# rostin79s/TFHE-AES

Hardware: AMD Instinct MI355X
Metric: AES-128 CTR blocks/sec (FHE) (higher is better)
Workload: dtype u64+f64; 1 GPU; configs[2]: 128 CTR blocks per GPU, Server::aes_encrypt 10 rounds (1280 bit-CBS/block), counters pre-incremented client-side; params=PARAM_OPT, blocks_per_gpu=128, total_blocks=128

## Files before the change

include/fheaes.h:

```cpp
#ifndef FHEAES_H
#define FHEAES_H

#include <stddef.h>
#include <stdint.h>

#ifdef __cplusplus
extern "C" {
#endif

#define FHEAES_OK 0
#define FHEAES_ERR_INVALID -1
#define FHEAES_ERR_NOKEYS -2
#define FHEAES_ERR_DEVICE -3
#define FHEAES_ERR_NOMEM -4

#define FHEAES_HOST 0
#define FHEAES_DEVICE 1

typedef struct fheaes_params {
    uint32_t lwe_dimension;
    uint32_t glwe_dimension;
    uint32_t polynomial_size;
    uint32_t pbs_base_log;
    uint32_t pbs_level;
// ... 85 lines not shown
size_t fheaes_packed_words(const fheaes_ctx *ctx, uint64_t m);
int fheaes_pack_bits(fheaes_ctx *ctx, const uint64_t *lwe_in, uint64_t m, uint64_t *glwe_out, int memspace);
int fheaes_unpack_bits(fheaes_ctx *ctx, const uint64_t *glwe_in, uint64_t m, uint64_t *lwe_out, int memspace);

int fheaes_expand_lwe_seeded(fheaes_ctx *ctx, const uint32_t *mask_key, uint64_t first_index, const uint64_t *bodies, uint64_t m,
                             uint64_t *lwe_out, int memspace);

size_t fheaes_packed_words_mod(const fheaes_ctx *ctx, uint64_t m, uint32_t width);
int fheaes_packed_mod_switch(fheaes_ctx *ctx, const uint64_t *glwe_in, uint64_t n_glwe, uint32_t width, uint64_t *out, int memspace);
int fheaes_pack_bits_mod(fheaes_ctx *ctx, const uint64_t *lwe_in, uint64_t m, uint32_t width, uint64_t *out, int memspace);
int fheaes_unpack_bits_mod(fheaes_ctx *ctx, const uint64_t *in, uint64_t m, uint32_t width, uint64_t *lwe_out, int memspace);

#define FHEAES_STAGE_KEYSWITCH 0
#define FHEAES_STAGE_BLIND_ROTATE 1
#define FHEAES_STAGE_PFPKS 2
#define FHEAES_STAGE_GGSW_FFT 3
#define FHEAES_STAGE_VERTICAL_PACKING 4
#define FHEAES_STAGE_LINEAR 5
#define FHEAES_STAGE_COUNT 6
int fheaes_profile_enable(fheaes_ctx *ctx, int on);
int fheaes_profile_reset(fheaes_ctx *ctx);
int fheaes_profile_read(fheaes_ctx *ctx, int stage, double *total_ms, uint64_t *launches, uint64_t *units);

int fheaes_get_twiddles(double *psi_out);
int fheaes_read_bsk_fourier(fheaes_ctx *ctx, uint32_t i, double *out);
int fheaes_k2_launch_plan(uint64_t m, uint32_t cu_count, uint32_t k, int *form, uint64_t *units_main, uint32_t *r_main,
                          uint64_t *units_tail, uint32_t *r_tail);
int fheaes_k2_launch_plan_forms(uint64_t m, uint32_t cu_count, uint32_t k, int allow_pair, int *form, uint64_t *units_main, uint32_t *r_main,
                                uint64_t *units_tail, uint32_t *r_tail);
int fheaes_k2_context_plan(fheaes_ctx *ctx, uint64_t m, int *form, uint64_t *units_main, uint32_t *r_main, uint64_t *units_tail,
                           uint32_t *r_tail, char *kernel, size_t kernel_cap);
int fheaes_k2_set_parking(fheaes_ctx *ctx, int claimed);
int fheaes_k2_set_forms(fheaes_ctx *ctx, int allow_pair, int allow_home);
#define FHEAES_K2_PARK_SLOTS 1024
int fheaes_k2_park_debug(fheaes_ctx *ctx, const uint32_t *initial_owner, int record);
int fheaes_k2_park_read(fheaes_ctx *ctx, uint64_t *fallbacks, uint64_t *violations, uint32_t *owner_out, uint32_t *record_out,
                        uint64_t record_cap, uint64_t *record_n);
const char *fheaes_version(void);

#ifdef __cplusplus
}
#endif
#endif
```

tfhe_aes_amd/_native.py:

```python
from __future__ import annotations

import ctypes
import os
import re
from pathlib import Path

import numpy as np

from . import _build
from .params import CParams, WopbsParameters

HOST, DEVICE = 0, 1
K2_PARK_SLOTS = 1024
STAGES = ("keyswitch", "blind_rotate", "pfpks", "ggsw_fft", "vertical_packing", "linear")

_u64p = ctypes.POINTER(ctypes.c_uint64)
_dp = ctypes.POINTER(ctypes.c_double)
_u32p = ctypes.POINTER(ctypes.c_uint32)
_ctx = ctypes.c_void_p
_c = ctypes

SIGNATURES = {
    "fheaes_create": (_c.c_int, [_c.POINTER(CParams), _c.c_int, _c.POINTER(_ctx)]),
    "fheaes_destroy": (None, [_ctx]),
    "fheaes_last_error": (_c.c_char_p, [_ctx]),
    "fheaes_key_words": (_c.c_size_t, [_ctx, _c.c_int]),
    "fheaes_upload_keys": (_c.c_int, [_ctx, _c.c_void_p, _c.c_void_p, _c.c_void_p, _c.c_int]),
    "fheaes_key_body_words": (_c.c_size_t, [_ctx, _c.c_int]),
    "fheaes_upload_keys_seeded": (_c.c_int, [_ctx, _c.POINTER(_c.c_uint32), _c.c_void_p, _c.c_void_p, _c.c_void_p, _c.c_int]),
    "fheaes_clone_keys": (_c.c_int, [_ctx, _ctx]),
    "fheaes_clone_info": (_c.c_int, [_ctx, _c.POINTER(_c.c_int), _u64p, _dp]),
    "fheaes_noise_level_seen": (_c.c_int, [_ctx, _c.POINTER(_c.c_uint32), _c.POINTER(_c.c_uint32)]),
    "fheaes_set_stream": (_c.c_int, [_ctx, _c.c_void_p]),
    "fheaes_synchronize": (_c.c_int, [_ctx]),
    "fheaes_reserve": (_c.c_int, [_ctx, _c.c_uint64]),
    "fheaes_keyswitch_batch": (_c.c_int, [_ctx, _c.c_void_p, _c.c_uint64, _c.c_void_p, _c.c_int]),
    "fheaes_cbs_pbs_batch": (_c.c_int, [_ctx, _c.c_void_p, _c.c_uint64, _c.c_uint32, _c.c_void_p, _c.c_int]),
    "fheaes_pfpks_batch": (_c.c_int, [_ctx, _c.c_void_p, _c.c_uint64, _c.c_void_p, _c.c_int]),
    "fheaes_forward_fourier_batch": (_c.c_int, [_ctx, _c.c_void_p, _c.c_uint64, _c.c_void_p, _c.c_int]),
    "fheaes_vertical_packing_batch": (_c.c_int, [_ctx, _c.c_void_p, _c.c_uint64, _c.c_uint32, _c.c_void_p, _c.c_uint32,
                                                 _c.c_int, _c.c_void_p, _c.c_int]),
    "fheaes_wopbs_batch": (_c.c_int, [_ctx, _c.c_void_p, _c.c_uint64, _c.c_uint32, _c.c_void_p, _c.c_uint32, _c.c_int,
                                      _c.c_void_p, _c.c_int]),
    "fheaes_gen_lut": (_c.c_int, [_c.c_uint32, _u64p, _u64p]),
    "fheaes_sbox": (_c.c_int, [_ctx, _c.c_void_p, _c.c_uint64, _c.c_int, _c.c_int]),
# ... 10 lines not shown
    "fheaes_aes_decrypt_equivalent_bits": (_c.c_int, [_ctx, _c.c_void_p, _c.c_uint32, _c.c_void_p, _c.c_uint64, _c.c_int]),
    "fheaes_add_scalar": (_c.c_int, [_ctx, _c.c_void_p, _c.c_uint64, _u64p, _c.c_int]),
    "fheaes_aes_encrypt_public_bits": (_c.c_int, [_ctx, _c.c_void_p, _c.c_uint32, _u64p, _c.c_uint64, _c.c_void_p, _c.c_int]),
    "fheaes_aes_ctr_bits": (_c.c_int, [_ctx, _c.c_void_p, _c.c_uint32, _u64p, _c.c_uint64, _u64p, _c.c_uint64, _c.c_void_p, _c.c_int]),
    "fheaes_aes_public_plan": (_c.c_int, [_u64p, _c.c_uint64, _c.c_uint32, _u64p]),
    "fheaes_aes_key_expansion_batch": (_c.c_int, [_ctx, _c.c_void_p, _c.c_uint32, _c.c_uint64, _c.c_void_p, _c.c_int]),
    "fheaes_aes_decryption_round_keys_batch": (_c.c_int, [_ctx, _c.c_void_p, _c.c_uint32, _c.c_uint64, _c.c_void_p, _c.c_int]),
    "fheaes_aes_encrypt_keyed": (_c.c_int, [_ctx, _c.c_void_p, _c.c_uint32, _c.c_uint64, _u32p, _c.c_void_p, _c.c_uint64, _c.c_int]),
    "fheaes_aes_decrypt_keyed": (_c.c_int, [_ctx, _c.c_void_p, _c.c_uint32, _c.c_uint64, _u32p, _c.c_void_p, _c.c_uint64, _c.c_int]),
    "fheaes_aes_decrypt_equivalent_keyed": (_c.c_int, [_ctx, _c.c_void_p, _c.c_uint32, _c.c_uint64, _u32p, _c.c_void_p, _c.c_uint64, _c.c_int]),
    "fheaes_aes_public_keyed": (_c.c_int, [_ctx, _c.c_void_p, _c.c_uint32, _c.c_uint64, _u32p, _u64p, _u64p, _c.c_uint64, _c.c_void_p, _c.c_int]),
    "fheaes_aes_public_plan_keyed": (_c.c_int, [_u64p, _u32p, _c.c_uint64, _c.c_uint64, _c.c_uint32, _u64p]),
    "fheaes_packed_words": (_c.c_size_t, [_ctx, _c.c_uint64]),
    "fheaes_pack_bits": (_c.c_int, [_ctx, _c.c_void_p, _c.c_uint64, _c.c_void_p, _c.c_int]),
    "fheaes_unpack_bits": (_c.c_int, [_ctx, _c.c_void_p, _c.c_uint64, _c.c_void_p, _c.c_int]),
    "fheaes_expand_lwe_seeded": (_c.c_int, [_ctx, _u32p, _c.c_uint64, _c.c_void_p, _c.c_uint64, _c.c_void_p, _c.c_int]),
    "fheaes_packed_words_mod": (_c.c_size_t, [_ctx, _c.c_uint64, _c.c_uint32]),
    "fheaes_packed_mod_switch": (_c.c_int, [_ctx, _c.c_void_p, _c.c_uint64, _c.c_uint32, _c.c_void_p, _c.c_int]),
    "fheaes_pack_bits_mod": (_c.c_int, [_ctx, _c.c_void_p, _c.c_uint64, _c.c_uint32, _c.c_void_p, _c.c_int]),
    "fheaes_unpack_bits_mod": (_c.c_int, [_ctx, _c.c_void_p, _c.c_uint64, _c.c_uint32, _c.c_void_p, _c.c_int]),
    "fheaes_profile_enable": (_c.c_int, [_ctx, _c.c_int]),
    "fheaes_profile_reset": (_c.c_int, [_ctx]),
    "fheaes_profile_read": (_c.c_int, [_ctx, _c.c_int, _dp, _u64p, _u64p]),
    "fheaes_get_twiddles": (_c.c_int, [_dp]),
    "fheaes_read_bsk_fourier": (_c.c_int, [_ctx, _c.c_uint32, _dp]),
    "fheaes_k2_launch_plan": (_c.c_int, [_c.c_uint64, _c.c_uint32, _c.c_uint32, _c.POINTER(_c.c_int), _c.POINTER(_c.c_uint64), _c.POINTER(_c.c_uint32),
                                       _c.POINTER(_c.c_uint64), _c.POINTER(_c.c_uint32)]),
    "fheaes_k2_launch_plan_forms": (_c.c_int, [_c.c_uint64, _c.c_uint32, _c.c_uint32, _c.c_int, _c.POINTER(_c.c_int), _c.POINTER(_c.c_uint64),
                                             _c.POINTER(_c.c_uint32), _c.POINTER(_c.c_uint64), _c.POINTER(_c.c_uint32)]),
    "fheaes_k2_context_plan": (_c.c_int, [_ctx, _c.c_uint64, _c.POINTER(_c.c_int), _c.POINTER(_c.c_uint64), _c.POINTER(_c.c_uint32),
                                        _c.POINTER(_c.c_uint64), _c.POINTER(_c.c_uint32), _c.c_char_p, _c.c_size_t]),
    "fheaes_k2_set_parking": (_c.c_int, [_ctx, _c.c_int]),
    "fheaes_k2_set_forms": (_c.c_int, [_ctx, _c.c_int, _c.c_int]),
    "fheaes_k2_park_debug": (_c.c_int, [_ctx, _c.POINTER(_c.c_uint32), _c.c_int]),
    "fheaes_k2_park_read": (_c.c_int, [_ctx, _u64p, _u64p, _c.POINTER(_c.c_uint32), _c.POINTER(_c.c_uint32), _c.c_uint64, _u64p]),
    "fheaes_version": (_c.c_char_p, []),
}

_lib = None


def header_symbols() -> list[str]:
    text = (_build.ROOT / "include" / "fheaes.h").read_text()
    text = re.sub(r"/\*.*?\*/", "", text, flags=re.S)
    return sorted(set(re.findall(r"\b(fheaes_[a-z0-9_]+)\s*\(", text)))


def load_library(build: bool = True):
    global _lib
    if _lib is not None:
        return _lib
    path = _build.build_engine() if build else _build.ENGINE_SO
    try:
        import torch
    except ImportError:
        pass
    if not Path(path).exists():
        raise RuntimeError("libfheaes.so is missing: run __graft_entry__.build() (hipcc --offload-arch=gfx950)")
    lib = ctypes.CDLL(str(path))
    for name, (res, args) in SIGNATURES.items():
        fn = getattr(lib, name)
        fn.restype, fn.argtypes = res, args
    _lib = lib
    return lib


# ... 230 lines not shown
    def pack_bits_mod(self, lwe_in, m: int, width: int, out):
        self._check(self._lib.fheaes_pack_bits_mod(self._h, _ptr(lwe_in)[0], m, width, _ptr(out)[0], self._space(lwe_in, out)))

    def unpack_bits_mod(self, packed_in, m: int, width: int, lwe_out):
        self._check(self._lib.fheaes_unpack_bits_mod(self._h, _ptr(packed_in)[0], m, width, _ptr(lwe_out)[0], self._space(packed_in, lwe_out)))

    def profile_enable(self, on: bool = True):
        self._check(self._lib.fheaes_profile_enable(self._h, int(on)))

    def profile_reset(self):
        self._check(self._lib.fheaes_profile_reset(self._h))

    def profile_read(self) -> dict:
        out = {}
        for i, name in enumerate(STAGES):
            ms, launches, units = ctypes.c_double(), ctypes.c_uint64(), ctypes.c_uint64()
            self._check(self._lib.fheaes_profile_read(self._h, i, ctypes.byref(ms), ctypes.byref(launches), ctypes.byref(units)))
            out[name] = {"ms": ms.value, "launches": launches.value, "units": units.value}
        return out

    def k2_plan(self, bits: int) -> dict:
        form, um, rm, ut, rt = _c.c_int(), _c.c_uint64(), _c.c_uint32(), _c.c_uint64(), _c.c_uint32()
        name = _c.create_string_buffer(96)
        self._check(self._lib.fheaes_k2_context_plan(self._h, bits, _c.byref(form), _c.byref(um), _c.byref(rm), _c.byref(ut), _c.byref(rt), name, len(name)))
        return {"form": form.value, "kernel": name.value.decode(), "units_main": um.value, "r_main": rm.value,
                "units_tail": ut.value, "r_tail": rt.value}

    def k2_set_parking(self, claimed: bool):
        self._check(self._lib.fheaes_k2_set_parking(self._h, 1 if claimed else 0))

    def k2_set_forms(self, allow_pair: bool = True, allow_home: bool = True):
        self._check(self._lib.fheaes_k2_set_forms(self._h, 1 if allow_pair else 0, 1 if allow_home else 0))

    def k2_park_debug(self, initial=None, record: bool = False):
        ptr = None
        if initial is not None:
            pat = np.ascontiguousarray(np.asarray(initial, dtype=np.uint32))
            if pat.shape != (K2_PARK_SLOTS,):
                raise ValueError("initial owner words: expected %d, got shape %s" % (K2_PARK_SLOTS, pat.shape))
            ptr = pat.ctypes.data_as(_c.POINTER(_c.c_uint32))
        self._check(self._lib.fheaes_k2_park_debug(self._h, ptr, 1 if record else 0))

    def k2_park_read(self) -> dict:
        fb, vi, n = _c.c_uint64(), _c.c_uint64(), _c.c_uint64()
        u32p = _c.POINTER(_c.c_uint32)
        self._check(self._lib.fheaes_k2_park_read(self._h, None, None, None, None, 0, _c.byref(n)))
        owner = np.zeros(K2_PARK_SLOTS, dtype=np.uint32)
        rec = np.zeros((n.value, 2), dtype=np.uint32)
        self._check(self._lib.fheaes_k2_park_read(self._h, _c.byref(fb), _c.byref(vi), owner.ctypes.data_as(u32p), rec.ctypes.data_as(u32p),
                                                  n.value, _c.byref(n)))
        return {"fallbacks": fb.value, "violations": vi.value, "owner": owner, "record": rec[:n.value]}

    def read_bsk_fourier(self, i: int) -> np.ndarray:
        p = self.params
        out = np.empty((p.pbs_level, p.k + 1, p.k + 1, 256, 2), dtype=np.float64)
        self._check(self._lib.fheaes_read_bsk_fourier(self._h, i, out.ctypes.data_as(_dp)))
        return out


def u128_pairs(values) -> np.ndarray:
    out = np.zeros((len(values), 2), dtype=np.uint64)
    for i, v in enumerate(values):
        if isinstance(v, (bytes, bytearray)):
            if len(v) != 16:
                raise ValueError("an AES block has 16 bytes, got %d" % len(v))
            v = int.from_bytes(v, "big")
# ... 4 lines not shown
    return out


def key_indices(key_of_block, n_blocks: int) -> np.ndarray:
    idx = [int(k) for k in key_of_block]
    if len(idx) != n_blocks:
        raise ValueError("one key index per block expected: %d for %d blocks" % (len(idx), n_blocks))
    if any(not 0 <= k < 1 << 32 for k in idx):
        raise ValueError("a key index is a uint32")
    out = np.zeros(max(n_blocks, 1), dtype=np.uint32)
    out[:n_blocks] = idx
    return out


def aes_public_plan_keyed(blocks, key_of_block, n_keys: int, key_bits: int = 128) -> list[int]:
    cnt = u128_pairs(blocks)
    kob = key_indices(key_of_block, len(cnt))
    out = np.zeros(14, dtype=np.uint64)
    rc = load_library().fheaes_aes_public_plan_keyed(cnt.ctypes.data_as(_u64p), kob.ctypes.data_as(_u32p), len(cnt), n_keys, key_bits, out.ctypes.data_as(_u64p))
    if rc != 0:
        raise FheAesError(rc, "fheaes_aes_public_plan_keyed: key_bits must be 128, 192 or 256, n_keys in 1..65536 and every key index below n_keys")
    return [int(x) for x in out[:{128: 10, 192: 12, 256: 14}[key_bits]]]


def aes_public_plan(blocks, key_bits: int = 128) -> list[int]:
    cnt = u128_pairs(blocks)
    out = np.zeros(14, dtype=np.uint64)
    rc = load_library().fheaes_aes_public_plan(cnt.ctypes.data_as(_u64p), len(cnt), key_bits, out.ctypes.data_as(_u64p))
    if rc != 0:
        raise FheAesError(rc, "fheaes_aes_public_plan: key_bits must be 128, 192 or 256")
    return [int(x) for x in out[:{128: 10, 192: 12, 256: 14}[key_bits]]]


def get_twiddles() -> np.ndarray:
    out = np.empty((512, 2), dtype=np.float64)
    rc = load_library().fheaes_get_twiddles(out.ctypes.data_as(_dp))
    if rc != 0:
        raise FheAesError(rc, "fheaes_get_twiddles")
    return out


def gen_lut(nb_block: int, f_table) -> np.ndarray:
    f = np.ascontiguousarray(f_table, dtype=np.uint64)
    if f.size != 1 << nb_block:
        raise ValueError("f_table must have 2^nb_block entries")
    out = np.empty((nb_block, max(512, 1 << nb_block)), dtype=np.uint64)
    rc = load_library().fheaes_gen_lut(nb_block, f.ctypes.data_as(_u64p), out.ctypes.data_as(_u64p))
    if rc != 0:
        raise FheAesError(rc, "fheaes_gen_lut")
    return out
```

tfhe_aes_amd/csrc/aes_schedule.h:

```cpp
#pragma once

static int many_sbox_dev(fheaes_ctx *c, const uint64_t *bytes, uint64_t n_bytes, int set, uint64_t *out)
{
    return wopbs_dev(c, bytes, n_bytes, 8, c->lutset_d[set], (uint32_t)c->lutset_n[set], 0, out);
}

static int aes_rounds(uint32_t key_bits) { return key_bits == 128 ? 10 : key_bits == 192 ? 12 : key_bits == 256 ? 14 : 0; }

static int check_key_bits(fheaes_ctx *c, uint32_t key_bits)
{
    if (!aes_rounds(key_bits)) return c->fail(FHEAES_ERR_INVALID, "key_bits must be 128, 192 or 256, got %u", key_bits);
    return FHEAES_OK;
}

static int aes_encrypt_dev(fheaes_ctx *c, const KeySets &rk, uint64_t *state, uint64_t n_blocks, int nr)
{
    const uint64_t bw = 8ull * c->big1, sw = 16 * bw, nbytes = 16 * n_blocks;
    TRY(ensure(c, c->ws_vp, nbytes * 3 * bw * 8));
    uint64_t *vp = (uint64_t *)c->ws_vp.p;
    const GatherTable t_round = table_enc_round(), t_shift = table_shift_rows(false);
    TRY(launch_add_bcast(c, state, rk, sw, n_blocks));
    for (int round = 1; round < nr; ++round) {
        TRY(many_sbox_dev(c, state, nbytes, LUTSET_ENC_ROUND, vp));
        TRY(launch_gather(c, vp, 3, rk.round(round, sw), state, n_blocks, t_round));
    }
    TRY(many_sbox_dev(c, state, nbytes, LUTSET_SBOX, vp));
    TRY(launch_gather(c, vp, 1, rk.round(nr, sw), state, n_blocks, t_shift));
    return FHEAES_OK;
}

static int aes_decrypt_dev(fheaes_ctx *c, const KeySets &rk, uint64_t *state, uint64_t n_blocks, int nr)
{
    const uint64_t bw = 8ull * c->big1, sw = 16 * bw, nbytes = 16 * n_blocks;
    TRY(ensure(c, c->ws_vp, nbytes * 4 * bw * 8));
    uint64_t *vp = (uint64_t *)c->ws_vp.p;
    const GatherTable t_inv = table_shift_rows(true), t_mix = table_dec_mix();
    const KeySets no_key{nullptr, nullptr, 0};
    TRY(launch_add_bcast(c, state, rk.round(nr, sw), sw, n_blocks));
    for (int round = nr; round >= 2; --round) {
        TRY(many_sbox_dev(c, state, nbytes, LUTSET_INV_SBOX, vp));
        TRY(launch_gather(c, vp, 1, rk.round(round - 1, sw), state, n_blocks, t_inv));
        TRY(many_sbox_dev(c, state, nbytes, LUTSET_DEC_MUL, vp));
        TRY(launch_gather(c, vp, 4, no_key, state, n_blocks, t_mix));
    }
    TRY(many_sbox_dev(c, state, nbytes, LUTSET_INV_SBOX, vp));
    TRY(launch_gather(c, vp, 1, rk, state, n_blocks, t_inv));
    return FHEAES_OK;
}

static int aes_decrypt_eq_dev(fheaes_ctx *c, const KeySets &dw, uint64_t *state, uint64_t n_blocks, int nr)
{
    const uint64_t bw = 8ull * c->big1, sw = 16 * bw, nbytes = 16 * n_blocks;
    TRY(ensure(c, c->ws_vp, nbytes * 4 * bw * 8));
    uint64_t *vp = (uint64_t *)c->ws_vp.p;
    const GatherTable t_round = table_dec_eq_round(), t_inv = table_shift_rows(true);
    TRY(launch_add_bcast(c, state, dw.round(nr, sw), sw, n_blocks));
    for (int round = nr - 1; round >= 1; --round) {
        TRY(many_sbox_dev(c, state, nbytes, LUTSET_DEC_EQ_ROUND, vp));
        TRY(launch_gather(c, vp, 4, dw.round(round, sw), state, n_blocks, t_round));
    }
    TRY(many_sbox_dev(c, state, nbytes, LUTSET_INV_SBOX, vp));
    TRY(launch_gather(c, vp, 1, dw, state, n_blocks, t_inv));
    return FHEAES_OK;
}

typedef int (*AesDevFn)(fheaes_ctx *, const KeySets &, uint64_t *, uint64_t, int);

static int dec_round_keys_dev(fheaes_ctx *c, const uint64_t *w, uint64_t *dw, int nr, uint64_t n_keys)
{
    const uint64_t bw = 8ull * c->big1, sw = 16 * bw, ks = (uint64_t)(nr + 1) * sw, mid = (uint64_t)(nr - 1) * 16, nbytes = mid * n_keys;
    const bool strided = n_keys > 1;
    TRY(ensure(c, c->ws_vp, nbytes * 4 * bw * 8));
    TRY(ensure(c, c->ws_tmp_a, nbytes * bw * 8));
    if (strided) TRY(ensure(c, c->ws_tmp_b, nbytes * bw * 8));
    uint64_t *vp = (uint64_t *)c->ws_vp.p, *mix = (uint64_t *)c->ws_tmp_a.p, *flat = (uint64_t *)c->ws_tmp_b.p;
    TRY(launch_key_rows(c, dw, ks, w, ks, 0, nullptr, 0, 0, 16, n_keys, 1));
    TRY(launch_key_rows(c, dw + (uint64_t)nr * sw, ks, w + (uint64_t)nr * sw, ks, 0, nullptr, 0, 0, 16, n_keys, 1));
    if (strided) TRY(launch_key_rows(c, flat, mid * bw, w + sw, ks, 0, nullptr, 0, 0, (uint32_t)mid, n_keys, 1));
    TRY(many_sbox_dev(c, strided ? flat : w + sw, nbytes, LUTSET_DEC_MUL, vp));
    TRY(launch_gather(c, vp, 4, KeySets{nullptr, nullptr, 0}, mix, nbytes / 16, table_dec_mix()));
    TRY(many_sbox_dev(c, mix, nbytes, LUTSET_IDENTITY, strided ? flat : dw + sw));
    if (strided) TRY(launch_key_rows(c, dw + sw, ks, flat, mid * bw, 0, nullptr, 0, 0, (uint32_t)mid, n_keys, 1));
    return FHEAES_OK;
}

static int key_expansion_dev(fheaes_ctx *c, const uint64_t *key, uint64_t *w, int nr, uint64_t n_keys)
{
    static const uint8_t RCON[10] = {0x01, 0x02, 0x04, 0x08, 0x10, 0x20, 0x40, 0x80, 0x1B, 0x36};
    const uint64_t bw = 8ull * c->big1, ww = 4 * bw, ks = (uint64_t)(nr + 1) * 16 * bw;
    const int nk = nr - 6;
    const bool strided = n_keys > 1;
    TRY(ensure(c, c->ws_tmp_a, n_keys * ww * 8));
    TRY(ensure(c, c->ws_tmp_b, n_keys * ww * 8));
    if (strided) TRY(ensure(c, c->ws_tmp_c, n_keys * ww * 8));
    uint64_t *ta = (uint64_t *)c->ws_tmp_a.p, *tb = (uint64_t *)c->ws_tmp_b.p, *tc = (uint64_t *)c->ws_tmp_c.p;
    TRY(launch_key_rows(c, w, ks, key, (uint64_t)nk * ww, 0, nullptr, 0, 0, 4u * nk, n_keys, 1));
    for (int i = nk; i < 4 * (nr + 1); ++i) {
// ... 181 lines not shown
```

tfhe_aes_amd/csrc/engine.hip:

```cpp
#include <hip/hip_runtime.h>
#include <cmath>
#include <cstdarg>
#include <cstdio>
#include <atomic>
#include <chrono>
#include <cstring>
#include <mutex>
#include <string>
#include <type_traits>
#include <unordered_map>
#include <vector>

#include "knobs.h"
#include "fheaes.h"
#include "fft_dev.h"
#include "kern_extprod.h"
#include "kern_blindrot_latency.h"
#include "kern_blindrot16.h"
#include "kern_blindrot_pair.h"
#include "ks_launch.h"
#include "kern_linear.h"

#define FHEAES_VERSION_STR "fheaes-mi355x 0.4 (gfx950)" FHEAES_BUILD_KIND

// ... 39 lines not shown
    *form = pl.form; *units_main = pl.units_main; *r_main = pl.r_main; *units_tail = pl.units_tail; *r_tail = pl.r_tail;
    return FHEAES_OK;
}
int fheaes_k2_context_plan(fheaes_ctx *ctx, uint64_t m, int *form, uint64_t *units_main, uint32_t *r_main, uint64_t *units_tail,
                           uint32_t *r_tail, char *kernel, size_t kernel_cap)
{
    if (!ctx) return FHEAES_ERR_INVALID;
    CtxLock lock__(ctx);
    if (!form || !units_main || !r_main || !units_tail || !r_tail || m == 0) return ctx->fail(FHEAES_ERR_INVALID, "k2_context_plan: null output or empty batch");
    const K2Launch L = k2_launch(ctx, m);
    const K2Plan &pl = L.pl;
    *form = pl.form; *units_main = pl.units_main; *r_main = pl.r_main; *units_tail = pl.units_tail; *r_tail = pl.r_tail;
    if (kernel && kernel_cap) { std::strncpy(kernel, L.name, kernel_cap - 1); kernel[kernel_cap - 1] = 0; }
    return FHEAES_OK;
}
int fheaes_k2_set_parking(fheaes_ctx *ctx, int claimed)
{
    if (!ctx) return FHEAES_ERR_INVALID;
    CtxLock lock__(ctx);
    if (claimed != 0 && claimed != 1) return ctx->fail(FHEAES_ERR_INVALID, "k2_set_parking: 1 = claimed slots, 0 = one private slot per workgroup (got %d)", claimed);
    HIP_TRY(ctx, hipStreamSynchronize(ctx->stream));
    ctx->k2_park_claim = claimed;
    return FHEAES_OK;
}
int fheaes_k2_set_forms(fheaes_ctx *ctx, int allow_pair, int allow_home)
{
    if (!ctx) return FHEAES_ERR_INVALID;
    CtxLock lock__(ctx);
    if ((allow_pair != 0 && allow_pair != 1) || (allow_home != 0 && allow_home != 1))
        return ctx->fail(FHEAES_ERR_INVALID, "k2_set_forms: each of allow_pair, allow_home is 0 or 1 (got %d, %d)", allow_pair, allow_home);
    HIP_TRY(ctx, hipStreamSynchronize(ctx->stream));
    ctx->k2_deny_pair = allow_pair == 0;
    ctx->k2_deny_home = allow_home == 0;
    return FHEAES_OK;
}
int fheaes_k2_park_debug(fheaes_ctx *ctx, const uint32_t *initial_owner, int record)
{
    if (!ctx) return FHEAES_ERR_INVALID;
    CtxLock lock__(ctx);
    if (record != 0 && record != 1) return ctx->fail(FHEAES_ERR_INVALID, "k2_park_debug: record must be 0 or 1 (got %d)", record);
    HIP_TRY(ctx, hipSetDevice(ctx->device));
    HIP_TRY(ctx, hipStreamSynchronize(ctx->stream));
    if (initial_owner) {
        TRY(ensure(ctx, ctx->ws_park_pattern, BRP_PARK_SLOTS * sizeof(uint32_t)));
        HIP_TRY(ctx, hipMemcpy(ctx->ws_park_pattern.p, initial_owner, BRP_PARK_SLOTS * sizeof(uint32_t), hipMemcpyHostToDevice));
    }
    if (ctx->ws_park_owner.p)
        HIP_TRY(ctx, hipMemset((char *)ctx->ws_park_owner.p + PARK_RECORD_PTR_OFFSET, 0, sizeof(uint64_t)));
    ctx->k2_park_pattern = initial_owner != nullptr;
    ctx->k2_park_record = record == 1;
    ctx->k2_park_record_n = 0;
    return FHEAES_OK;
}
int fheaes_k2_park_read(fheaes_ctx *ctx, uint64_t *fallbacks, uint64_t *violations, uint32_t *owner_out, uint32_t *record_out,
                        uint64_t record_cap, uint64_t *record_n)
{
    if (!ctx) return FHEAES_ERR_INVALID;
    CtxLock lock__(ctx);
    if (record_out && record_cap < ctx->k2_park_record_n)
        return ctx->fail(FHEAES_ERR_INVALID, "k2_park_read: %llu records do not fit record_cap = %llu", (unsigned long long)ctx->k2_park_record_n,
                         (unsigned long long)record_cap);
    HIP_TRY(ctx, hipSetDevice(ctx->device));
    HIP_TRY(ctx, hipStreamSynchronize(ctx->stream));
    uint32_t words[PARK_OWNER_BYTES / sizeof(uint32_t)] = {};
    if (ctx->ws_park_owner.p) HIP_TRY(ctx, hipMemcpy(words, ctx->ws_park_owner.p, PARK_OWNER_BYTES, hipMemcpyDeviceToHost));
    uint64_t counters[2];
// ... 873 lines not shown
```

tfhe_aes_amd/csrc/engine_ctx.h:

```cpp
#pragma once

namespace {

std::string g_create_error;
thread_local std::string tl_error;
thread_local uint64_t tl_error_ctx_id = 0;
std::atomic<uint64_t> g_next_ctx_id{1};

}

struct DevBuf {
    void *p = nullptr;
    size_t bytes = 0;
    DevBuf() = default;
    DevBuf(const DevBuf &) = delete;
    DevBuf &operator=(const DevBuf &) = delete;
    ~DevBuf() { if (p) (void)hipFree(p); }
};

struct fheaes_ctx {
    fheaes_params p{};
    const uint64_t id = g_next_ctx_id.fetch_add(1);
    int device = 0;
    hipStream_t own_stream = nullptr, stream = nullptr;
    std::string err;
    std::recursive_mutex mu;
    uint32_t n = 0, k = 0, k1 = 0, big = 0, big1 = 0;
    uint32_t cu_count = 256;
    int clone_path = FHEAES_CLONE_NONE;
    uint64_t clone_bytes = 0;
    double clone_seconds = 0.0;
    uint32_t noise_level_seen = 0;
    int k2_home = -1;
    int k2_pair_ok = -1;
    bool k2_deny_pair = false, k2_deny_home = false;
    int k2_park_claim = 1;
    bool k2_park_pattern = false, k2_park_record = false;
    uint64_t k2_park_record_n = 0;
    int8_t *ksk_frag = nullptr, *pfpksk_frag = nullptr;
    uint32_t ks_ksteps = 0, ks_coltiles = 0, pf_ksteps = 0, pf_coltiles = 0;
    size_t ksk_frag_bytes = 0, pfpksk_frag_bytes = 0, bskf_bytes = 0;
    double2 *bskf = nullptr;
    bool have_keys = false;
    double2 *tw_d = nullptr;
    uint64_t *lutset_d[LUTSET_COUNT] = {};
    int lutset_n[LUTSET_COUNT] = {};
    DevBuf ws_small, ws_pbs, ws_ggsw, ws_ggswf, ws_vp, ws_tmp_a, ws_tmp_b, ws_tmp_c, ws_luts, ws_misc, ws_digits, ws_park, ws_park_owner, ws_tree;
    DevBuf ws_park_pattern, ws_park_record;
    DevBuf stage[4];
    uint8_t *pin = nullptr;
    size_t pin_bytes = 0;
    hipEvent_t pin_ev = nullptr;
    bool prof = false;
    struct Pending { hipEvent_t a, b; int stage; };
    std::vector<Pending> pending;
    std::vector<hipEvent_t> free_events;
    double stage_ms[FHEAES_STAGE_COUNT] = {};
    uint64_t stage_launches[FHEAES_STAGE_COUNT] = {};
    uint64_t stage_units[FHEAES_STAGE_COUNT] = {};

    int fail(int code, const char *fmt, ...)
    {
        char buf[512];
        va_list ap;
        va_start(ap, fmt);
        vsnprintf(buf, sizeof buf, fmt, ap);
        va_end(ap);
        err = buf;
        tl_error = buf;
        tl_error_ctx_id = id;
        return code;
// ... 145 lines not shown
```

tfhe_aes_amd/csrc/engine_launch.h:

```cpp
#pragma once

#define MAX_CHUNK_BITS 32768ull
#define MAX_WOPBS_BITS 16u

namespace {

#define LATENCY_BATCH_BITS 256ull
#define K2_PAIR_MIN_BITS 768ull
struct K2Plan { int form; uint64_t units_main; uint32_t r_main; uint64_t units_tail; uint32_t r_tail; };
K2Plan k2_plan(uint64_t m, uint32_t cu_count, uint32_t k1, bool allow_pair = true)
{
    K2Plan pl{};
    if (m <= LATENCY_BATCH_BITS) { pl.form = 0; pl.units_main = m; pl.r_main = 1; return pl; }
    if (allow_pair && k1 == 5 && m > K2_PAIR_MIN_BITS) {
        pl.form = 2; pl.r_main = 6; pl.r_tail = 4;
        const uint64_t gens = (m + 6ull * cu_count - 1) / (6ull * cu_count);
        uint64_t nu = gens * cu_count;
        uint64_t four = 6 * nu >= m ? (6 * nu - m) / 2 : 0;
        if (four > nu) four = nu;
        if (four == nu && 4 * nu > m) { nu = (m + 3) / 4; four = nu; }
        pl.units_tail = four; pl.units_main = nu - four;
        return pl;
    }
    pl.form = 1;
    pl.r_main = k1 == 5 ? 3 : 8;
    pl.units_main = (m + pl.r_main - 1) / pl.r_main;
    if (k1 == 5) {
        const uint64_t slots = 2ull * cu_count;
        pl.r_tail = 2;
        if ((m + 1) / 2 <= cu_count) {
            pl.units_main = 0;
            pl.units_tail = (m + 1) / 2;
        } else if (pl.units_main > slots) {
            const uint64_t nu = slots * ((m + 3 * slots - 1) / (3 * slots));
            if (2 * nu <= m) {
                pl.units_tail = 3 * nu - m;
                pl.units_main = nu - pl.units_tail;
            }
        }
    }
    return pl;
}

int launch_keyswitch(fheaes_ctx *c, const uint64_t *in, uint64_t m, uint64_t *out)
{
    if (m == 0) return FHEAES_OK;
    StageScope sc(c, FHEAES_STAGE_KEYSWITCH, m);
    const uint64_t ct_tiles16 = ((m + KS_CT_TILE - 1) / KS_CT_TILE) * (KS_CT_TILE / 16);
    TRY(ensure(c, c->ws_digits, ct_tiles16 * c->ks_ksteps * 1024));
    int8_t *af = (int8_t *)c->ws_digits.p;
    const uint64_t threads = ct_tiles16 * c->ks_ksteps * 64;
    ks_launch_digits_k1(dim3((unsigned)((threads + 255) / 256)), c->stream, in, (uint64_t)c->big1, c->big, m, c->ks_ksteps, af);
    KeyswitchArgs a{};
    a.afrag = af; a.bfrag = c->ksk_frag; a.ksteps = c->ks_ksteps; a.coltiles = c->ks_coltiles;
    a.in = in; a.in_stride = c->big1; a.body_index = (int32_t)c->big; a.body_col = c->n; a.ncols = c->n + 1;
    a.out = out; a.out_stride = c->n + 1; a.out_z_stride = 0; a.m = m;
    dim3 grid((c->ks_coltiles + KSL_COL_TILES - 1) / KSL_COL_TILES, (unsigned)((m + 16 * KSL_CT_TILES - 1) / (16 * KSL_CT_TILES)), 1);
    ks_launch_mfma_lds(1, grid, c->stream, a);
    HIP_TRY(c, hipGetLastError());
    return FHEAES_OK;
}

int launch_pfpks(fheaes_ctx *c, const uint64_t *in, uint64_t m, uint64_t *out, uint64_t out_stride, int block = -1)
{
    if (m == 0) return FHEAES_OK;
    StageScope sc(c, FHEAES_STAGE_PFPKS, m);
    const uint32_t gsz = c->k1 * FHE_N;
    const uint64_t ct_tiles16 = ((m + KS_CT_TILE - 1) / KS_CT_TILE) * (KS_CT_TILE / 16);
    TRY(ensure(c, c->ws_digits, ct_tiles16 * c->pf_ksteps * 2 * 1024));
    int8_t *af = (int8_t *)c->ws_digits.p;
    const uint64_t threads = ct_tiles16 * c->pf_ksteps * 64;
    ks_launch_digits_k3(dim3((unsigned)((threads + 255) / 256)), c->stream, in, (uint64_t)c->big1, c->big1, m, c->pf_ksteps, af);
    KeyswitchArgs a{};
// ... 60 lines not shown
}

struct K2Launch {
    K2Plan pl;
    void (*kernel)(ExtProdArgs);
    const char *name;
    unsigned grid, threads;
    size_t park_bytes;
    bool park_owner;
};
K2Launch k2_launch(fheaes_ctx *c, uint64_t m)
{
    K2Launch L{};
    L.pl = k2_plan(m, c->cu_count, c->k1, k2_pair_allowed(c));
    L.grid = (unsigned)(L.pl.units_main + L.pl.units_tail);
    if (L.pl.form == 0) {
        L.threads = BL_THREADS;
        if (c->k1 == 5) { L.kernel = blind_rotate_latency_kernel<5, 5, 8>; L.name = "blind_rotate_latency_kernel<5,5,8>"; }
        else { L.kernel = blind_rotate_latency_kernel<2, 5, 8>; L.name = "blind_rotate_latency_kernel<2,5,8>"; }
    } else if (L.pl.form == 2) {
        L.threads = BRP_THREADS;
        L.kernel = blind_rotate_pair_kernel<5, 5, 8, 3, 2>;
        L.name = c->k2_park_claim ? "blind_rotate_pair_kernel<5,5,8,3,2> parking=claimed" : "blind_rotate_pair_kernel<5,5,8,3,2> parking=private";
        L.park_bytes = k2_pair_park_bytes(c, L.grid);
        L.park_owner = c->k2_park_claim != 0;
    } else {
        L.threads = EP_THREADS;
        if (c->k1 == 5 && k2_home_allowed(c)) { L.kernel = blind_rotate16_kernel<5, 5, 8, 3, 2, true>; L.name = "blind_rotate16_kernel<5,5,8,3,2,true>"; }
        else if (c->k1 == 5) { L.kernel = blind_rotate16_kernel<5, 5, 8, 3, 2, false>; L.name = "blind_rotate16_kernel<5,5,8,3,2,false>"; }
        else { L.kernel = blind_rotate16_kernel<2, 5, 8, 8>; L.name = "blind_rotate16_kernel<2,5,8,8,0,false>"; }
        L.park_bytes = (size_t)L.grid * BR16_PARK_WORDS_PER_WG * 8;
    }
    return L;
}

int launch_cbs_pbs(fheaes_ctx *c, const uint64_t *lwe_small, uint64_t m, uint32_t level, uint64_t *out)
{
    if (m == 0) return FHEAES_OK;
    if ((uint64_t)c->n * c->p.pbs_level * c->k1 * c->k1 * FHE_H * 16 > 0x7FFFFFFFull)
        return c->fail(FHEAES_ERR_INVALID, "bootstrapping key larger than 2 GiB is not supported by the blind-rotation kernels");
    StageScope sc(c, FHEAES_STAGE_BLIND_ROTATE, m);
    ExtProdArgs a{};
    a.ggsw = c->bskf; a.tw = c->tw_d;
    a.out = out; a.count = m; a.iters = c->n; a.lwe_in = lwe_small;
    const uint64_t half_delta = 1ull << (64 - c->p.cbs_base_log * level - 1);
    a.tv_const = (uint64_t)0 - half_delta; a.body_shift = 1ull << 62; a.post_add = half_delta;
    const K2Launch L = k2_launch(c, m);
    if (L.pl.form != 0) a.units_main = (uint32_t)L.pl.units_main;
    if (L.park_bytes) {
        if (L.park_bytes > 0x7FFFFFFFull) return c->fail(FHEAES_ERR_INVALID, "internal: parking slab of %zu bytes exceeds one raw buffer", L.park_bytes);
        TRY(ensure(c, c->ws_park, L.park_bytes));
        a.park = (uint64_t *)c->ws_park.p; a.park_bytes = L.park_bytes;
    }
    if (L.park_owner) {
        TRY(ensure_park_owner(c));
        if (c->k2_park_pattern)
            HIP_TRY(c, hipMemcpyAsync(c->ws_park_owner.p, c->ws_park_pattern.p, BRP_PARK_SLOTS * sizeof(uint32_t), hipMemcpyDeviceToDevice, c->stream));
        else
            HIP_TRY(c, hipMemsetAsync(c->ws_park_owner.p, 0, BRP_PARK_SLOTS * sizeof(uint32_t), c->stream));
        a.park_owner = (uint32_t *)c->ws_park_owner.p;
        if (c->k2_park_record) {
            TRY(ensure(c, c->ws_park_record, (size_t)L.grid * 2 * sizeof(uint32_t)));
            HIP_TRY(c, hipMemsetAsync(c->ws_park_record.p, 0xFF, (size_t)L.grid * 2 * sizeof(uint32_t), c->stream));
            const uint64_t rp = (uint64_t)(uintptr_t)c->ws_park_record.p;
            uint32_t *const rp_word = (uint32_t *)((char *)c->ws_park_owner.p + PARK_RECORD_PTR_OFFSET);
            HIP_TRY(c, hipMemsetD32Async((hipDeviceptr_t)rp_word, (int)(uint32_t)rp, 1, c->stream));
// ... 243 lines not shown
```

Baseline: 57.91 blocks/s.

## Window AES bootstraps across round boundaries to fill blind-rotation waves

Folds the encrypt and decrypt round loops into one step schedule. Bootstraps then run in fixed-size windows of block-steps that may span two consecutive AES steps, with the window sized to a multiple of the blind-rotation generation width. The planner uses windowing only when it cuts the total number of pair-kernel generations compared with per-round batching. The goal is to remove partly empty final waves on the GPU, at the cost of extra keyswitch, vertical-packing and gather launches when a window straddles two steps.

Result: faster. 58.62 blocks/s (median of 6 runs) (+1.2%).

```diff
diff --git a/include/fheaes.h b/include/fheaes.h
--- a/include/fheaes.h
+++ b/include/fheaes.h
@@ -141,6 +141,11 @@
                            uint32_t *r_tail, char *kernel, size_t kernel_cap);
 int fheaes_k2_set_parking(fheaes_ctx *ctx, int claimed);
 int fheaes_k2_set_forms(fheaes_ctx *ctx, int allow_pair, int allow_home);
+int fheaes_aes_window_plan(uint64_t n_blocks, uint32_t steps, uint32_t cu_count, uint32_t k, uint64_t *window_blocks, uint64_t *launches,
+                           uint64_t *generations, uint64_t *generations_by_round);
+int fheaes_aes_context_window(fheaes_ctx *ctx, uint64_t n_blocks, uint32_t steps, uint64_t *window_blocks);
+#define FHEAES_AES_WINDOW_OFF 0xFFFFFFFFu
+int fheaes_aes_set_window(fheaes_ctx *ctx, uint32_t window_blocks);
 #define FHEAES_K2_PARK_SLOTS 1024
 int fheaes_k2_park_debug(fheaes_ctx *ctx, const uint32_t *initial_owner, int record);
 int fheaes_k2_park_read(fheaes_ctx *ctx, uint64_t *fallbacks, uint64_t *violations, uint32_t *owner_out, uint32_t *record_out,
diff --git a/tfhe_aes_amd/_native.py b/tfhe_aes_amd/_native.py
--- a/tfhe_aes_amd/_native.py
+++ b/tfhe_aes_amd/_native.py
@@ -11,6 +11,7 @@
 from .params import CParams, WopbsParameters
 
 HOST, DEVICE = 0, 1
+AES_WINDOW_OFF = 0xFFFFFFFF
 K2_PARK_SLOTS = 1024
 STAGES = ("keyswitch", "blind_rotate", "pfpks", "ggsw_fft", "vertical_packing", "linear")
 
@@ -87,6 +88,9 @@
                                         _c.POINTER(_c.c_uint64), _c.POINTER(_c.c_uint32), _c.c_char_p, _c.c_size_t]),
     "fheaes_k2_set_parking": (_c.c_int, [_ctx, _c.c_int]),
     "fheaes_k2_set_forms": (_c.c_int, [_ctx, _c.c_int, _c.c_int]),
+    "fheaes_aes_window_plan": (_c.c_int, [_c.c_uint64, _c.c_uint32, _c.c_uint32, _c.c_uint32, _u64p, _u64p, _u64p, _u64p]),
+    "fheaes_aes_context_window": (_c.c_int, [_ctx, _c.c_uint64, _c.c_uint32, _u64p]),
+    "fheaes_aes_set_window": (_c.c_int, [_ctx, _c.c_uint32]),
     "fheaes_k2_park_debug": (_c.c_int, [_ctx, _c.POINTER(_c.c_uint32), _c.c_int]),
     "fheaes_k2_park_read": (_c.c_int, [_ctx, _u64p, _u64p, _c.POINTER(_c.c_uint32), _c.POINTER(_c.c_uint32), _c.c_uint64, _u64p]),
     "fheaes_version": (_c.c_char_p, []),
@@ -383,6 +387,14 @@
     def k2_set_forms(self, allow_pair: bool = True, allow_home: bool = True):
         self._check(self._lib.fheaes_k2_set_forms(self._h, 1 if allow_pair else 0, 1 if allow_home else 0))
 
+    def aes_window(self, n_blocks: int, steps: int) -> int:
+        w = _c.c_uint64()
+        self._check(self._lib.fheaes_aes_context_window(self._h, n_blocks, steps, _c.byref(w)))
+        return w.value
+
+    def aes_set_window(self, window_blocks: int = 0):
+        self._check(self._lib.fheaes_aes_set_window(self._h, int(window_blocks)))
+
     def k2_park_debug(self, initial=None, record: bool = False):
         ptr = None
         if initial is not None:
@@ -453,6 +465,14 @@
     return [int(x) for x in out[:{128: 10, 192: 12, 256: 14}[key_bits]]]
 
 
+def aes_window_plan(n_blocks: int, steps: int, cu_count: int = 256, k: int = 4) -> dict:
+    w, la, g, gr = _c.c_uint64(), _c.c_uint64(), _c.c_uint64(), _c.c_uint64()
+    rc = load_library().fheaes_aes_window_plan(n_blocks, steps, cu_count, k, _c.byref(w), _c.byref(la), _c.byref(g), _c.byref(gr))
+    if rc != 0:
+        raise FheAesError(rc, "fheaes_aes_window_plan: n_blocks, steps and cu_count must be at least 1")
+    return {"window": w.value, "launches": la.value, "generations": g.value, "generations_by_round": gr.value}
+
+
 def get_twiddles() -> np.ndarray:
     out = np.empty((512, 2), dtype=np.float64)
     rc = load_library().fheaes_get_twiddles(out.ctypes.data_as(_dp))
diff --git a/tfhe_aes_amd/csrc/aes_schedule.h b/tfhe_aes_amd/csrc/aes_schedule.h
--- a/tfhe_aes_amd/csrc/aes_schedule.h
+++ b/tfhe_aes_amd/csrc/aes_schedule.h
@@ -13,56 +13,99 @@
     return FHEAES_OK;
 }
 
-static int aes_encrypt_dev(fheaes_ctx *c, const KeySets &rk, uint64_t *state, uint64_t n_blocks, int nr)
-{
-    const uint64_t bw = 8ull * c->big1, sw = 16 * bw, nbytes = 16 * n_blocks;
-    TRY(ensure(c, c->ws_vp, nbytes * 3 * bw * 8));
+struct AesStep { int set; uint32_t n_luts; GatherTable table; int key_round; };
+struct AesSchedule {
+    int first_key_round = 0;
+    uint32_t max_luts = 0;
+    std::vector<AesStep> steps;
+    void add(int set, uint32_t n_luts, const GatherTable &t, int key_round) { steps.push_back({set, n_luts, t, key_round}); max_luts = std::max(max_luts, n_luts); }
+};
+
+static AesSchedule aes_encrypt_schedule(int nr)
+{
+    AesSchedule s;
+    s.first_key_round = 0;
+    for (int round = 1; round < nr; ++round) s.add(LUTSET_ENC_ROUND, 3, table_enc_round(), round);
+    s.add(LUTSET_SBOX, 1, table_shift_rows(false), nr);
+    return s;
+}
+
+static AesSchedule aes_decrypt_schedule(int nr)
+{
+    AesSchedule s;
+    s.first_key_round = nr;
+    for (int round = nr; round >= 2; --round) {
+        s.add(LUTSET_INV_SBOX, 1, table_shift_rows(true), round - 1);
+        s.add(LUTSET_DEC_MUL, 4, table_dec_mix(), -1);
+    }
+    s.add(LUTSET_INV_SBOX, 1, table_shift_rows(true), 0);
+    return s;
+}
+
+static AesSchedule aes_decrypt_eq_schedule(int nr)
+{
+    AesSchedule s;
+    s.first_key_round = nr;
+    for (int round = nr - 1; round >= 1; --round) s.add(LUTSET_DEC_EQ_ROUND, 4, table_dec_eq_round(), round);
+    s.add(LUTSET_INV_SBOX, 1, table_shift_rows(true), 0);
+    return s;
+}
+
+static int aes_run_dev(fheaes_ctx *c, const KeySets &rk, uint64_t *state, uint64_t n_blocks, const AesSchedule &sch)
+{
+    const uint64_t bw = 8ull * c->big1, sw = 16 * bw, steps = sch.steps.size();
+    auto key_of = [&](const AesStep &st, uint64_t first_block) {
+        if (st.key_round < 0) return KeySets{nullptr, nullptr, 0};
+        return KeySets{rk.rk + (uint64_t)st.key_round * sw, rk.of_block ? rk.of_block + first_block : nullptr, rk.stride};
+    };
+    const uint64_t w = aes_context_window(c, n_blocks, steps);
+    TRY(ensure(c, c->ws_vp, (w ? w : n_blocks) * 16 * sch.max_luts * bw * 8));
     uint64_t *vp = (uint64_t *)c->ws_vp.p;
-    const GatherTable t_round = table_enc_round(), t_shift = table_shift_rows(false);
-    TRY(launch_add_bcast(c, state, rk, sw, n_blocks));
-    for (int round = 1; round < nr; ++round) {
-        TRY(many_sbox_dev(c, state, nbytes, LUTSET_ENC_ROUND, vp));
-        TRY(launch_gather(c, vp, 3, rk.round(round, sw), state, n_blocks, t_round));
-    }
-    TRY(many_sbox_dev(c, state, nbytes, LUTSET_SBOX, vp));
-    TRY(launch_gather(c, vp, 1, rk.round(nr, sw), state, n_blocks, t_shift));
-    return FHEAES_OK;
-}
-
-static int aes_decrypt_dev(fheaes_ctx *c, const KeySets &rk, uint64_t *state, uint64_t n_blocks, int nr)
-{
-    const uint64_t bw = 8ull * c->big1, sw = 16 * bw, nbytes = 16 * n_blocks;
-    TRY(ensure(c, c->ws_vp, nbytes * 4 * bw * 8));
-    uint64_t *vp = (uint64_t *)c->ws_vp.p;
-    const GatherTable t_inv = table_shift_rows(true), t_mix = table_dec_mix();
-    const KeySets no_key{nullptr, nullptr, 0};
-    TRY(launch_add_bcast(c, state, rk.round(nr, sw), sw, n_blocks));
-    for (int round = nr; round >= 2; --round) {
-        TRY(many_sbox_dev(c, state, nbytes, LUTSET_INV_SBOX, vp));
-        TRY(launch_gather(c, vp, 1, rk.round(round - 1, sw), state, n_blocks, t_inv));
-        TRY(many_sbox_dev(c, state, nbytes, LUTSET_DEC_MUL, vp));
-        TRY(launch_gather(c, vp, 4, no_key, state, n_blocks, t_mix));
-    }
-    TRY(many_sbox_dev(c, state, nbytes, LUTSET_INV_SBOX, vp));
-    TRY(launch_gather(c, vp, 1, rk, state, n_blocks, t_inv));
-    return FHEAES_OK;
-}
-
-static int aes_decrypt_eq_dev(fheaes_ctx *c, const KeySets &dw, uint64_t *state, uint64_t n_blocks, int nr)
-{
-    const uint64_t bw = 8ull * c->big1, sw = 16 * bw, nbytes = 16 * n_blocks;
-    TRY(ensure(c, c->ws_vp, nbytes * 4 * bw * 8));
-    uint64_t *vp = (uint64_t *)c->ws_vp.p;
-    const GatherTable t_round = table_dec_eq_round(), t_inv = table_shift_rows(true);
-    TRY(launch_add_bcast(c, state, dw.round(nr, sw), sw, n_blocks));
-    for (int round = nr - 1; round >= 1; --round) {
-        TRY(many_sbox_dev(c, state, nbytes, LUTSET_DEC_EQ_ROUND, vp));
-        TRY(launch_gather(c, vp, 4, dw.round(round, sw), state, n_blocks, t_round));
-    }
-    TRY(many_sbox_dev(c, state, nbytes, LUTSET_INV_SBOX, vp));
-    TRY(launch_gather(c, vp, 1, dw, state, n_blocks, t_inv));
-    return FHEAES_OK;
-}
+    TRY(launch_add_bcast(c, state, rk.round((uint64_t)sch.first_key_round, sw), sw, n_blocks));
+    if (w == 0) {
+        for (const AesStep &st : sch.steps) {
+            TRY(many_sbox_dev(c, state, 16 * n_blocks, st.set, vp));
+            TRY(launch_gather(c, vp, st.n_luts, key_of(st, 0), state, n_blocks, st.table));
+        }
+        return FHEAES_OK;
+    }
+    const uint64_t ggsw_words = (uint64_t)c->k1 * c->k1 * FHE_N, total = steps * n_blocks;
+    TRY(ensure_wopbs_ws(c, w * AES_BLOCK_BITS));
+    uint64_t *small = (uint64_t *)c->ws_small.p, *pbs = (uint64_t *)c->ws_pbs.p, *ggsw = (uint64_t *)c->ws_ggsw.p;
+    const double2 *ggswf = (const double2 *)c->ws_ggswf.p;
+    struct Segment { const AesStep *st; uint64_t first, blocks, row; uint64_t *vp; };
+    for (uint64_t i0 = 0; i0 < total; i0 += w) {
+        const uint64_t len = std::min<uint64_t>(w, total - i0), s = i0 / n_blocks, b0 = i0 % n_blocks, m = len * AES_BLOCK_BITS;
+        Segment seg[2] = {{&sch.steps[s], b0, std::min<uint64_t>(len, n_blocks - b0), 0, vp}, {}};
+        int n_seg = 1;
+        if (seg[0].blocks < len) {
+            seg[1] = {&sch.steps[s + 1], 0, len - seg[0].blocks, seg[0].blocks, vp + seg[0].blocks * 16 * seg[0].st->n_luts * bw};
+            n_seg = 2;
+        }
+        for (int g = 0; g < n_seg; ++g)
+            TRY(launch_keyswitch(c, state + seg[g].first * sw, seg[g].blocks * AES_BLOCK_BITS, small + seg[g].row * AES_BLOCK_BITS * (c->n + 1)));
+        TRY(launch_cbs_pbs(c, small, m, 1, pbs));
+        TRY(launch_pfpks(c, pbs, m, ggsw, ggsw_words));
+        TRY(launch_forward_fourier(c, ggsw, m * c->k1 * c->k1, (double2 *)c->ws_ggswf.p, FHEAES_STAGE_GGSW_FFT));
+        if (n_seg == 1 || seg[0].st->set == seg[1].st->set) {
+            const int set = seg[0].st->set;
+            TRY(launch_vertical_packing(c, ggswf, 16 * len, 8, c->lutset_d[set], (uint32_t)c->lutset_n[set], 0, vp));
+        } else {
+            for (int g = 0; g < n_seg; ++g) {
+                const int set = seg[g].st->set;
+                TRY(launch_vertical_packing(c, ggswf + seg[g].row * AES_BLOCK_BITS * (ggsw_words / 2), 16 * seg[g].blocks, 8, c->lutset_d[set],
+                                            (uint32_t)c->lutset_n[set], 0, seg[g].vp));
+            }
+        }
+        for (int g = 0; g < n_seg; ++g)
+            TRY(launch_gather(c, seg[g].vp, seg[g].st->n_luts, key_of(*seg[g].st, seg[g].first), state + seg[g].first * sw, seg[g].blocks, seg[g].st->table));
+    }
+    return FHEAES_OK;
+}
+
+static int aes_encrypt_dev(fheaes_ctx *c, const KeySets &rk, uint64_t *state, uint64_t n_blocks, int nr) { return aes_run_dev(c, rk, state, n_blocks, aes_encrypt_schedule(nr)); }
+static int aes_decrypt_dev(fheaes_ctx *c, const KeySets &rk, uint64_t *state, uint64_t n_blocks, int nr) { return aes_run_dev(c, rk, state, n_blocks, aes_decrypt_schedule(nr)); }
+static int aes_decrypt_eq_dev(fheaes_ctx *c, const KeySets &dw, uint64_t *state, uint64_t n_blocks, int nr) { return aes_run_dev(c, dw, state, n_blocks, aes_decrypt_eq_schedule(nr)); }
 
 typedef int (*AesDevFn)(fheaes_ctx *, const KeySets &, uint64_t *, uint64_t, int);
 
diff --git a/tfhe_aes_amd/csrc/engine.hip b/tfhe_aes_amd/csrc/engine.hip
--- a/tfhe_aes_amd/csrc/engine.hip
+++ b/tfhe_aes_amd/csrc/engine.hip
@@ -95,6 +95,30 @@
     HIP_TRY(ctx, hipStreamSynchronize(ctx->stream));
     ctx->k2_deny_pair = allow_pair == 0;
     ctx->k2_deny_home = allow_home == 0;
+    return FHEAES_OK;
+}
+int fheaes_aes_window_plan(uint64_t n_blocks, uint32_t steps, uint32_t cu_count, uint32_t k, uint64_t *window_blocks, uint64_t *launches,
+                           uint64_t *generations, uint64_t *generations_by_round)
+{
+    if (!window_blocks || !launches || !generations || !generations_by_round || n_blocks == 0 || steps == 0 || cu_count == 0) return FHEAES_ERR_INVALID;
+    const AesWindowPlan pl = aes_window_plan(n_blocks, steps, cu_count, k + 1);
+    *window_blocks = pl.window; *launches = pl.launches; *generations = pl.generations; *generations_by_round = pl.generations_by_round;
+    return FHEAES_OK;
+}
+int fheaes_aes_context_window(fheaes_ctx *ctx, uint64_t n_blocks, uint32_t steps, uint64_t *window_blocks)
+{
+    if (!ctx) return FHEAES_ERR_INVALID;
+    CtxLock lock__(ctx);
+    if (!window_blocks) return ctx->fail(FHEAES_ERR_INVALID, "aes_context_window: null output");
+    *window_blocks = aes_context_window(ctx, n_blocks, steps);
+    return FHEAES_OK;
+}
+int fheaes_aes_set_window(fheaes_ctx *ctx, uint32_t window_blocks)
+{
+    if (!ctx) return FHEAES_ERR_INVALID;
+    CtxLock lock__(ctx);
+    HIP_TRY(ctx, hipStreamSynchronize(ctx->stream));
+    ctx->aes_window = window_blocks;
     return FHEAES_OK;
 }
 int fheaes_k2_park_debug(fheaes_ctx *ctx, const uint32_t *initial_owner, int record)
diff --git a/tfhe_aes_amd/csrc/engine_ctx.h b/tfhe_aes_amd/csrc/engine_ctx.h
--- a/tfhe_aes_amd/csrc/engine_ctx.h
+++ b/tfhe_aes_amd/csrc/engine_ctx.h
@@ -37,6 +37,7 @@
     int k2_park_claim = 1;
     bool k2_park_pattern = false, k2_park_record = false;
     uint64_t k2_park_record_n = 0;
+    uint32_t aes_window = 0;
     int8_t *ksk_frag = nullptr, *pfpksk_frag = nullptr;
     uint32_t ks_ksteps = 0, ks_coltiles = 0, pf_ksteps = 0, pf_coltiles = 0;
     size_t ksk_frag_bytes = 0, pfpksk_frag_bytes = 0, bskf_bytes = 0;
diff --git a/tfhe_aes_amd/csrc/engine_launch.h b/tfhe_aes_amd/csrc/engine_launch.h
--- a/tfhe_aes_amd/csrc/engine_launch.h
+++ b/tfhe_aes_amd/csrc/engine_launch.h
@@ -39,6 +39,48 @@
             }
         }
     }
+    return pl;
+}
+
+#define AES_BLOCK_BITS 128ull
+#define AES_WINDOW_MAX_BLOCKS (MAX_CHUNK_BITS / AES_BLOCK_BITS)
+struct AesWindowPlan { uint64_t window, launches, generations, generations_by_round; };
+
+uint64_t k2_generations(uint64_t m, uint32_t cu_count, uint32_t k1)
+{
+    if (m == 0) return 0;
+    if (m <= K2_PAIR_MIN_BITS) return 1;
+    const K2Plan pl = k2_plan(m, cu_count, k1);
+    return (pl.units_main + pl.units_tail + cu_count - 1) / cu_count;
+}
+
+void aes_window_count(uint64_t n, uint64_t steps, uint64_t w, uint32_t cu_count, uint32_t k1, uint64_t *launches, uint64_t *generations)
+{
+    const uint64_t total = steps * n, full = total / w, rest = total % w;
+    *launches = full + (rest ? 1 : 0);
+    *generations = full * k2_generations(w * AES_BLOCK_BITS, cu_count, k1) + k2_generations(rest * AES_BLOCK_BITS, cu_count, k1);
+}
+
+AesWindowPlan aes_window_plan(uint64_t n, uint64_t steps, uint32_t cu_count, uint32_t k1, bool allow_pair = true)
+{
+    AesWindowPlan pl{};
+    const uint64_t chunks = n / AES_WINDOW_MAX_BLOCKS, last = n % AES_WINDOW_MAX_BLOCKS;
+    pl.launches = steps * (chunks + (last ? 1 : 0));
+    pl.generations_by_round = steps * (chunks * k2_generations(MAX_CHUNK_BITS, cu_count, k1) + k2_generations(last * AES_BLOCK_BITS, cu_count, k1));
+    pl.generations = pl.generations_by_round;
+    if (n == 0 || steps == 0) return pl;
+    const uint64_t gen_bits = 6ull * cu_count;
+    if (k2_plan(std::min<uint64_t>(n * AES_BLOCK_BITS, MAX_CHUNK_BITS), cu_count, k1, allow_pair).form != 2) return pl;
+    if (n * AES_BLOCK_BITS % gen_bits == 0) return pl;
+    uint64_t g = AES_BLOCK_BITS, r = gen_bits;
+    while (r) { const uint64_t t = g % r; g = r; r = t; }
+    const uint64_t base = gen_bits / g;
+    const uint64_t w = std::min<uint64_t>(n, AES_WINDOW_MAX_BLOCKS) / base * base;
+    if (w == 0) return pl;
+    uint64_t launches, generations;
+    aes_window_count(n, steps, w, cu_count, k1, &launches, &generations);
+    if (generations >= pl.generations_by_round) return pl;
+    pl.window = w; pl.launches = launches; pl.generations = generations;
     return pl;
 }
 
@@ -165,6 +207,14 @@
         L.park_bytes = (size_t)L.grid * BR16_PARK_WORDS_PER_WG * 8;
     }
     return L;
+}
+
+uint64_t aes_context_window(fheaes_ctx *c, uint64_t n, uint64_t steps)
+{
+    if (n == 0 || steps == 0 || c->aes_window == FHEAES_AES_WINDOW_OFF) return 0;
+    if (c->aes_window) return std::min<uint64_t>(c->aes_window, std::min<uint64_t>(n, AES_WINDOW_MAX_BLOCKS));
+    const bool pair = k2_launch(c, std::min<uint64_t>(n * AES_BLOCK_BITS, MAX_CHUNK_BITS)).pl.form == 2;
+    return aes_window_plan(n, steps, c->cu_count, c->k1, pair).window;
 }
 
 int launch_cbs_pbs(fheaes_ctx *c, const uint64_t *lwe_small, uint64_t m, uint32_t level, uint64_t *out)
```
